# yoshitomo-matsubara/hnd-ghnd-object-detectors

Hardware: AMD Instinct MI355X
Metric: distill-step images/sec at 3x800x1333, GHND Faster R-CNN b3ch (higher is better)
Workload: dtype f32

## Files before the change

### hnd_ghnd_object_detectors_amd/csrc/conv_bx3.hip

```cpp

#include "bf16x3.h"
#include "common.h"

#include <stdlib.h>

namespace {

using hnd::bf8;
using hnd::cu_count;
using hnd::f32x4;
using hnd::FastDiv;
using hnd::split_pair;
using hnd::static_for;
using hnd::u32x4;

struct Bx3Args {
  FastDiv div_ow, div_oh;
  int nsl;
  int nchunks;
  int mrows;
  int cpg;
  int res_up;
};

template <int OFF>
__device__ __forceinline__ void rload(f32x4& dst, const float* p) {
  asm volatile("global_load_dwordx4 %0, %1, off offset:%2" : "=a"(dst) : "v"(p), "n"(OFF));
}
template <int CNT>
__device__ __forceinline__ void rwait(f32x4& a0, f32x4& a1, f32x4& a2, f32x4& a3, f32x4& a4, f32x4& a5, f32x4& a6,
                                      f32x4& a7) {
  asm volatile("s_waitcnt vmcnt(%8)"
               : "+a"(a0), "+a"(a1), "+a"(a2), "+a"(a3), "+a"(a4), "+a"(a5), "+a"(a6), "+a"(a7)
               : "n"(CNT));
}

__device__ __forceinline__ void bload(uint32_t& dst, const uint8_t* p) {
  asm volatile("global_load_ubyte %0, %1, off" : "=a"(dst) : "v"(p));
}
template <int CNT>
__device__ __forceinline__ void bwait8(uint32_t& a0, uint32_t& a1, uint32_t& a2, uint32_t& a3, uint32_t& a4, uint32_t& a5,
                                       uint32_t& a6, uint32_t& a7) {
  asm volatile("s_waitcnt vmcnt(%8)"
               : "+a"(a0), "+a"(a1), "+a"(a2), "+a"(a3), "+a"(a4), "+a"(a5), "+a"(a6), "+a"(a7)
               : "n"(CNT));
}

template <int CNT>
__device__ __forceinline__ void rwait8(f32x4& a0, f32x4& a1, f32x4& a2, f32x4& a3, f32x4& a4, f32x4& a5, f32x4& a6,
                                       f32x4& a7) {
  rwait<CNT>(a0, a1, a2, a3, a4, a5, a6, a7);
}

template <int KS, bool RES, bool MO, bool MK = false>
__global__ void __launch_bounds__(256, 1) bx3_kernel(const hnd_conv_desc d, const Bx3Args a) {
  static_assert(!MK || RES, "the mask build rides on the residual build's bookkeeping");
  constexpr int RESLOADS = RES ? (MK ? 32 : 16) : 0;
  constexpr int RING = RES ? 2 : 4, K = 32 * KS, MI = 4, NI = 4, PLANE = 64 * K, STORES = MO ? 32 : 16;
  static_assert(KS % RING == 0, "ring slots are compile-time: the ring must divide the k steps of a tile");
  extern __shared__ __attribute__((aligned(16))) uint16_t Bs[];
  const int tid = threadIdx.x, lane = tid & 63, wave = tid >> 6;
  const int l16 = lane & 15, g4 = lane >> 4;
  const int b = blockIdx.x, xcd = b & 7, idx = b >> 3, per_xcd = gridDim.x >> 3;
  const int slice = idx % a.nsl, tpx = per_xcd / a.nsl;
  const int team = xcd * tpx + idx / a.nsl, nteams = 8 * tpx;
  const int n0 = slice * 64;
  const int c_lo = (int)((long long)a.nchunks * team / nteams);
  const int c_hi = (int)((long long)a.nchunks * (team + 1) / nteams);

  auto a_ptr = [&](int cc, int mi) -> const float* {
    const unsigned m = min((unsigned)(cc * 64 + mi * 16 + l16), (unsigned)(a.mrows - 1));
    const unsigned t = hnd::fdiv(m, a.div_ow), ow_ = m - t * (unsigned)d.ow;
    const unsigned n_ = hnd::fdiv(t, a.div_oh), oh_ = t - n_ * (unsigned)d.oh;
    const size_t pix = ((size_t)n_ * d.h + oh_ * (unsigned)d.sh) * (size_t)d.w_ + ow_ * (unsigned)d.sw;
    return d.x + pix * (size_t)d.cin + (size_t)(g4 * 8);
  };
  const int col0 = n0 + l16 * 4;
  float es[NI], eb[NI];
#pragma unroll
  for (int ni = 0; ni < NI; ++ni) {
    es[ni] = d.epi_scale ? d.epi_scale[col0 + ni] : 1.f;
    eb[ni] = d.epi_shift ? d.epi_shift[col0 + ni] : 0.f;
  }
  const size_t slice_elems = (size_t)3 * PLANE;

  int c = c_lo;
  while (c < c_hi) {
    const int grp = a.cpg > 0 ? c / a.cpg : 0;
    const int seg_hi = a.cpg > 0 ? min(c_hi, (grp + 1) * a.cpg) : c_hi;
    __syncthreads();
    {
      const u32x4* src = (const u32x4*)(d.w_bf16x3 + ((size_t)grp * a.nsl + slice) * slice_elems);
      u32x4* dst = (u32x4*)Bs;
      constexpr int NV = 3 * PLANE / 8, UB = 12;
      static_assert(NV % (256 * UB) == 0, "slice does not divide among the threads");
#pragma unroll 1
      for (int i0 = 0; i0 < NV; i0 += 256 * UB) {
        u32x4 t[UB];
#pragma unroll
        for (int u = 0; u < UB; ++u) t[u] = src[i0 + u * 256 + tid];
#pragma unroll
        for (int u = 0; u < UB; ++u) dst[i0 + u * 256 + tid] = t[u];
      }
    }
    __syncthreads();

    int cc = c + wave;
    if (cc < seg_hi) {
      const float* aptr[MI];
      f32x4 ring[RING][MI][2];
#pragma unroll
      for (int mi = 0; mi < MI; ++mi) aptr[mi] = a_ptr(cc, mi);
      static_for<RING>([&](auto U) __attribute__((always_inline)) {
        constexpr int u = decltype(U)::value;
        static_for<MI>([&](auto I) __attribute__((always_inline)) {
          constexpr int mi = decltype(I)::value;
          rload<(u % KS) * 128>(ring[u][mi][0], aptr[mi]);
          rload<(u % KS) * 128 + 16>(ring[u][mi][1], aptr[mi]);
        });
      });
      uint32_t pl[2][3][MI][4];
      float dummy = 0.f;
#pragma unroll
      for (int i = 0; i < STORES; ++i) asm volatile("global_load_dword %0, %1, off" : "+v"(dummy) : "v"(aptr[0]));
      rwait<8 * (RING - 1) + STORES>(ring[0][0][0], ring[0][0][1], ring[0][1][0], ring[0][1][1], ring[0][2][0], ring[0][2][1],
                                     ring[0][3][0], ring[0][3][1]);
#pragma unroll
      for (int mi = 0; mi < MI; ++mi)
#pragma unroll
        for (int j = 0; j < 4; ++j) {
          const f32x4 v = ring[0][mi][j >> 1];
          const float x0 = (j & 1) ? v.z : v.x, x1 = (j & 1) ? v.w : v.y;
          split_pair(x0, x1, pl[0][0][mi][j], pl[0][1][mi][j], pl[0][2][mi][j]);
        }
      f32x4 acc[MI][NI];
      bf8 bfirst[3];
      {
        const uint16_t* br = Bs + l16 * K + ((g4 ^ l16) * 8);
        bfirst[0] = *(const bf8*)(br); bfirst[1] = *(const bf8*)(br + PLANE); bfirst[2] = *(const bf8*)(br + 2 * PLANE);
      }
      f32x4 resv[MI][4];
      uint32_t resm[MI][4];
      for (; cc < seg_hi; cc += 4) {
        const int cn = cc + 4 < seg_hi ? cc + 4 : cc;
        const float* nptr[MI];
#pragma unroll
        for (int mi = 0; mi < MI; ++mi) nptr[mi] = a_ptr(cn, mi);
        static_for<KS>([&](auto G) __attribute__((always_inline)) {
          constexpr int ks = decltype(G)::value, slot = ks % RING, par = ks & 1;
          constexpr int slot1 = (ks + 1) % RING;
          if constexpr (MK && ks == KS - 4) {
#pragma unroll
            for (int mi = 0; mi < MI; ++mi)
#pragma unroll
              for (int r = 0; r < 4; ++r)
                bload(resm[mi][r], d.mask_bits + (((size_t)min(cc * 64 + mi * 16 + g4 * 4 + r, a.mrows - 1) * (size_t)d.ldc + col0) >> 2));
          }
          if constexpr (RES && ks == KS - 4) {
#pragma unroll
            for (int mi = 0; mi < MI; ++mi) {
              const unsigned mr = (unsigned)(cc * 64 + mi * 16 + g4 * 4);
              const unsigned m0 = min(mr, (unsigned)(a.mrows - 4));
              const unsigned t = hnd::fdiv(m0, a.div_ow), ow_ = m0 - t * (unsigned)d.ow;
              const unsigned n_ = hnd::fdiv(t, a.div_oh), oh_ = t - n_ * (unsigned)d.oh;
              const size_t pu = ((size_t)n_ * d.res1_h + (oh_ >> 1)) * (size_t)d.res1_w + (ow_ >> 1);
              const bool up = a.res_up != 0;
              const unsigned ml = (unsigned)(a.mrows - 1);
              const size_t p0 = up ? pu : (size_t)min(mr, ml), p1 = up ? pu : (size_t)min(mr + 1, ml),
                           p2 = up ? pu + 1 : (size_t)min(mr + 2, ml), p3 = up ? pu + 1 : (size_t)min(mr + 3, ml);
              rload<0>(resv[mi][0], d.res1 + p0 * (size_t)d.ldc + col0);
              rload<0>(resv[mi][1], d.res1 + p1 * (size_t)d.ldc + col0);
              rload<0>(resv[mi][2], d.res1 + p2 * (size_t)d.ldc + col0);
              rload<0>(resv[mi][3], d.res1 + p3 * (size_t)d.ldc + col0);
            }
          }
          static_for<MI>([&](auto I) __attribute__((always_inline)) {
            constexpr int mi = decltype(I)::value;
            if constexpr (ks + RING < KS) {
              rload<(ks + RING) * 128>(ring[slot][mi][0], aptr[mi]);
              rload<(ks + RING) * 128 + 16>(ring[slot][mi][1], aptr[mi]);
            } else {
              rload<(ks + RING - KS) * 128>(ring[slot][mi][0], nptr[mi]);
              rload<(ks + RING - KS) * 128 + 16>(ring[slot][mi][1], nptr[mi]);
            }
          });
          constexpr int kResYounger = (RES && ks >= KS - 4 && ks <= KS - 4 + RING - 2) ? RESLOADS : 0;
          if constexpr (ks < RING - 1) {
            rwait<(8 * (RING - 1) + STORES + kResYounger < 63 ? 8 * (RING - 1) + STORES + kResYounger : 63)>(
                ring[slot1][0][0], ring[slot1][0][1], ring[slot1][1][0], ring[slot1][1][1], ring[slot1][2][0],
                ring[slot1][2][1], ring[slot1][3][0], ring[slot1][3][1]);
          } else {
            rwait<8 * (RING - 1) + kResYounger>(ring[slot1][0][0], ring[slot1][0][1], ring[slot1][1][0], ring[slot1][1][1],
                                                ring[slot1][2][0], ring[slot1][2][1], ring[slot1][3][0], ring[slot1][3][1]);
          }
          const int pos = ((ks * 4 + g4) ^ l16) * 8;
          bf8 bcur[3], bnxt[3];
          bcur[0] = bfirst[0]; bcur[1] = bfirst[1]; bcur[2] = bfirst[2];
          static_for<NI>([&](auto NIc) __attribute__((always_inline)) {
            constexpr int ni = decltype(NIc)::value;
            if constexpr (ni + 1 < NI) {
              const uint16_t* br = Bs + ((ni + 1) * 16 + l16) * K + pos;
              bnxt[0] = *(const bf8*)(br); bnxt[1] = *(const bf8*)(br + PLANE); bnxt[2] = *(const bf8*)(br + 2 * PLANE);
            } else {
              const uint16_t* br = Bs + l16 * K + ((((ks + 1) % KS) * 4 + g4) ^ l16) * 8;
              bfirst[0] = *(const bf8*)(br); bfirst[1] = *(const bf8*)(br + PLANE); bfirst[2] = *(const bf8*)(br + 2 * PLANE);
            }
            static_for<MI>([&](auto MIc) __attribute__((always_inline)) {
              constexpr int mi = decltype(MIc)::value;
              auto frag = [&](int q) __attribute__((always_inline)) {
                const u32x4 t = {pl[par][q][mi][0], pl[par][q][mi][1], pl[par][q][mi][2], pl[par][q][mi][3]};
                return __builtin_bit_cast(bf8, t);
              };
              const bf8 ah = frag(0), am = frag(1), al = frag(2);
              constexpr int p = ni * 4 + mi, rg = p >> 2, j = p & 3;
              const f32x4 v = ring[slot1][rg][j >> 1];
              const float x0 = (j & 1) ? v.z : v.x, x1 = (j & 1) ? v.w : v.y;
              f32x4 cacc = (ks == 0) ? f32x4{0.f, 0.f, 0.f, 0.f} : acc[mi][ni];
              cacc = __builtin_amdgcn_mfma_f32_16x16x32_bf16(al, bcur[0], cacc, 0, 0, 0);
              const uint32_t h0 = __float_as_uint(x0) & 0xffff0000u, h1 = __float_as_uint(x1) & 0xffff0000u;
              __builtin_amdgcn_sched_barrier(0);
              cacc = __builtin_amdgcn_mfma_f32_16x16x32_bf16(ah, bcur[2], cacc, 0, 0, 0);
              const float r0 = x0 - __uint_as_float(h0), r1 = x1 - __uint_as_float(h1);
              __builtin_amdgcn_sched_barrier(0);
              cacc = __builtin_amdgcn_mfma_f32_16x16x32_bf16(am, bcur[1], cacc, 0, 0, 0);
              const uint32_t m0 = __float_as_uint(r0) & 0xffff0000u, m1 = __float_as_uint(r1) & 0xffff0000u;
              __builtin_amdgcn_sched_barrier(0);
              cacc = __builtin_amdgcn_mfma_f32_16x16x32_bf16(am, bcur[0], cacc, 0, 0, 0);
              const float q0 = r0 - __uint_as_float(m0), q1 = r1 - __uint_as_float(m1);
              __builtin_amdgcn_sched_barrier(0);
              cacc = __builtin_amdgcn_mfma_f32_16x16x32_bf16(ah, bcur[1], cacc, 0, 0, 0);
              pl[par ^ 1][0][rg][j] = __builtin_amdgcn_perm(h1, h0, 0x07060302u);
              pl[par ^ 1][1][rg][j] = __builtin_amdgcn_perm(m1, m0, 0x07060302u);
              pl[par ^ 1][2][rg][j] = __builtin_amdgcn_perm(__float_as_uint(q1), __float_as_uint(q0), 0x07060302u);
              __builtin_amdgcn_sched_barrier(0);
              cacc = __builtin_amdgcn_mfma_f32_16x16x32_bf16(ah, bcur[0], cacc, 0, 0, 0);
              acc[mi][ni] = cacc;
              __builtin_amdgcn_sched_barrier(0);
            });
            if constexpr (ni + 1 < NI) { bcur[0] = bnxt[0]; bcur[1] = bnxt[1]; bcur[2] = bnxt[2]; }
          });
        });
        if constexpr (RES) {
          rwait8<32>(resv[0][0], resv[0][1], resv[0][2], resv[0][3], resv[1][0], resv[1][1], resv[1][2], resv[1][3]);
          rwait8<32>(resv[2][0], resv[2][1], resv[2][2], resv[2][3], resv[3][0], resv[3][1], resv[3][2], resv[3][3]);
          if constexpr (MK) {
            bwait8<32>(resm[0][0], resm[0][1], resm[0][2], resm[0][3], resm[1][0], resm[1][1], resm[1][2], resm[1][3]);
            bwait8<32>(resm[2][0], resm[2][1], resm[2][2], resm[2][3], resm[3][0], resm[3][1], resm[3][2], resm[3][3]);
          }
        }
#pragma unroll
        for (int mi = 0; mi < MI; ++mi)
#pragma unroll
          for (int r = 0; r < 4; ++r) {
            const size_t m = (size_t)min(cc * 64 + mi * 16 + g4 * 4 + r, a.mrows - 1);
            f32x4 v;
#pragma unroll
            for (int ni = 0; ni < NI; ++ni) {
              float x = acc[mi][ni][r] * es[ni] + eb[ni];
              if (RES) x += resv[mi][r][ni];
              if (MK) x = ((resm[mi][r] >> ni) & 1u) ? x : 0.f;
              v[ni] = d.relu ? fmaxf(x, 0.f) : x;
            }
            const size_t yo = m * (size_t)d.ldc + col0;
            *(f32x4*)(d.y + yo) = v;
            if (MO)
              d.mask_out[yo >> 2] = (uint8_t)((v[0] > 0.f ? 1 : 0) | (v[1] > 0.f ? 2 : 0) | (v[2] > 0.f ? 4 : 0) |
                                              (v[3] > 0.f ? 8 : 0));
          }
#pragma unroll
        for (int mi = 0; mi < MI; ++mi) aptr[mi] = nptr[mi];
      }
      asm volatile("s_waitcnt vmcnt(0)" : "+v"(dummy)::"memory");
    }
    c = seg_hi;
  }
}

__global__ void pack_bx3_kernel(const float* __restrict__ w, uint16_t* __restrict__ img, int rows_pad, int K, int KI, int groups,
                                long long group_stride, long long total) {
  const int nsl = rows_pad / 64;
  const size_t plane = (size_t)64 * KI;
  for (long long e = blockIdx.x * (long long)blockDim.x + threadIdx.x; e < total; e += (long long)gridDim.x * blockDim.x) {
    const int k = (int)(e % K);
    long long t = e / K;
    const int row = (int)(t % rows_pad), g = (int)(t / rows_pad);
    const float x = w[(size_t)g * (size_t)group_stride + (size_t)row * K + k];
    const uint32_t xb = __float_as_uint(x), hb = xb & 0xffff0000u;
    const float r1 = x - __uint_as_float(hb);
    const uint32_t mb = __float_as_uint(r1) & 0xffff0000u;
    const float r2 = r1 - __uint_as_float(mb);
    const int part = k / KI, kk = k - part * KI;
    const int s = row / 64, r = row % 64, c = kk >> 3, pos = c ^ (r & 15);
    uint16_t* o = img + (((size_t)part * groups + g) * nsl + s) * 3 * plane + (size_t)r * KI + pos * 8 + (kk & 7);
    o[0] = (uint16_t)(hb >> 16);
    o[plane] = (uint16_t)(mb >> 16);
    o[2 * plane] = (uint16_t)(__float_as_uint(r2) >> 16);
  }
}

template <int KS, bool RES, bool MO, bool MK = false>
int launch_bx3_t(const hnd_conv_desc& d, const Bx3Args& a, int grid, hipStream_t stream) {
  const size_t lds = (size_t)3 * 64 * 32 * KS * sizeof(uint16_t);
  return hnd::launch_big_lds<bx3_kernel<KS, RES, MO, MK>>(dim3(grid), dim3(256), lds, 160 * 1024, stream, "hnd_conv2d_igemm(bx3)",
                                                          d, a);
}

}

namespace hnd {

static bool bx3_recommended(long long rows_per_image, int kdim, int cout) {
  if (rows_per_image <= 0 || cout <= 0 || cout % 64 != 0) return false;
  if (kdim != 128 && (kdim % 256 != 0 || kdim > 2048)) return false;
  const long long nteams = team_count(cout, 64);
  if (nteams == 0) return false;
  const long long chunks_at_16 = (rows_per_image * 16 + 63) / 64;
  return chunks_at_16 / nteams >= (kdim > 512 ? 16 : 8);
}

bool bx3_applies(const hnd_conv_desc& d) {
  if (!d.w_bf16x3) return false;
  if (d.kh != 1 || d.kw != 1 || d.bh != 0 || d.bw != 0 || d.cin != d.kdim) return false;
  if (d.kdim != 128 && (d.kdim % 256 != 0 || d.kdim > 2048)) return false;
  if (d.stats || d.pro_scale || d.res2 || d.mask || d.bwd_x) return false;
  if (d.mask_bits && d.mask_out) return false;
  if (d.mask_bits && d.kdim <= 256 && (!d.res1 || d.res1_mode != 0)) return false;
  if (d.res1 && ((uintptr_t)d.res1 % 16) != 0) return false;
  if (d.res1 && d.res1_mode == 1 && (d.yh != 2 * d.res1_h || d.yw != 2 * d.res1_w || d.ow % 4 != 0)) return false;
  if (d.cout % 64 != 0 || d.ldc % 4 != 0 || ((uintptr_t)d.y % 16) != 0) return false;
  if (team_count(d.cout, 64) == 0) return false;
  if (d.y_sh != 1 || d.y_sw != 1 || d.y_oh != 0 || d.y_ow != 0 || d.yh != d.oh || d.yw != d.ow) return false;
  if (!samples_inside(d)) return false;
  const long long M = gemm_rows(d);
  if (M < 64 || d.w_group_rows % 64 != 0) return false;
  if (M % 64 != 0 && d.w_group_rows != 0) return false;
  return true;
}

static int launch_bx3_one(const hnd_conv_desc& d, int kpart, hipStream_t stream) {
  Bx3Args a;
  a.div_ow = make_fastdiv((unsigned)d.ow);
  a.div_oh = make_fastdiv((unsigned)d.oh);
  a.nsl = d.cout / 64;
  a.mrows = (int)gemm_rows(d);
  a.nchunks = (a.mrows + 63) / 64;
  a.cpg = d.w_group_rows / 64;
  a.res_up = d.res1 && d.res1_mode == 1;
  const int grid = (cu_count() / 8) * 8;
  if (d.mask_bits)
    return kpart == 128 ? launch_bx3_t<4, true, false, true>(d, a, grid, stream)
                        : launch_bx3_t<8, true, false, true>(d, a, grid, stream);
  const int sel = (kpart == 128 ? 0 : 4) | (d.res1 ? 2 : 0) | (d.mask_out ? 1 : 0);
  switch (sel) {
    case 0: return launch_bx3_t<4, false, false>(d, a, grid, stream);
    case 1: return launch_bx3_t<4, false, true>(d, a, grid, stream);
    case 2: return launch_bx3_t<4, true, false>(d, a, grid, stream);
    case 3: return launch_bx3_t<4, true, true>(d, a, grid, stream);
    case 4: return launch_bx3_t<8, false, false>(d, a, grid, stream);
    case 5: return launch_bx3_t<8, false, true>(d, a, grid, stream);
    case 6: return launch_bx3_t<8, true, false>(d, a, grid, stream);
    default: return launch_bx3_t<8, true, true>(d, a, grid, stream);
  }
}

int launch_bx3_tiled(const hnd_conv_desc& d, int mi, hipStream_t stream);

static const int BX3_TILED_BELOW_K128 = 3, BX3_TILED_BELOW_K256 = 3, BX3_TILED_BELOW_K512 = 10, BX3_TILED_BELOW_KLONG = 16;
static const int BX3_TILED_128_ROWS_FROM = 10;

int bx3_build(const hnd_conv_desc& d) {
  const long long chunks = (gemm_rows(d) + 63) / 64, nteams = team_count(d.cout, 64);
  const long long per_team = (chunks + nteams - 1) / nteams;
  const bool is_long = d.kdim >= 1024;
  const int rows = is_long && per_team >= BX3_TILED_128_ROWS_FROM ? 2 : 1;
  const int forced = debug_picker("bx3_tiled");
  if (forced >= 0) {
    const int mi = debug_picker("bx3_tiled_mi");
    return forced ? (mi == 1 || mi == 2 ? mi : rows) : 0;
  }
  if (d.w_group_rows > 0) return 0;
  const int below = d.kdim <= 128 ? BX3_TILED_BELOW_K128
                                  : (d.kdim <= 256 ? BX3_TILED_BELOW_K256 : (is_long ? BX3_TILED_BELOW_KLONG : BX3_TILED_BELOW_K512));
  return per_team < below ? rows : 0;
}

int launch_bx3(const hnd_conv_desc& d, int build, hipStream_t stream) {
  if (build) return launch_bx3_tiled(d, build, stream);
  if (d.kdim <= 256) return launch_bx3_one(d, d.kdim, stream);
  const long long groups = d.w_group_rows > 0 ? gemm_rows(d) / d.w_group_rows : 1;
  const int parts = d.kdim / 256;
  const size_t part_elems = (size_t)groups * (size_t)(d.cout / 64) * (size_t)3 * 64 * 256;
  for (int p = 0; p < parts; ++p) {
    hnd_conv_desc q = d;
    if (p + 1 < parts) {
      q.relu = 0;
      q.mask_out = nullptr;
      q.mask_bits = nullptr;
    }
    if (p > 0) {
      q.x = d.x + (size_t)256 * p;
      q.w_bf16x3 = d.w_bf16x3 + part_elems * (size_t)p;
      q.epi_shift = nullptr;
      q.res1 = d.y;
      q.res1_mode = 0;
    }
    const int rc = launch_bx3_one(q, 256, stream);
    if (rc) return rc;
  }
  return 0;
}

}

extern "C" int hnd_bf16x3_recommended(int64_t rows_per_image, int kdim, int cout) {
  return hnd::bx3_recommended((long long)rows_per_image, kdim, cout) ? 1 : 0;
}

extern "C" size_t hnd_pack_bf16x3_elems(int rows_pad, int kdim, int groups) {
  if (rows_pad <= 0 || rows_pad % 64 != 0 || kdim <= 0 || kdim % 8 != 0 || groups < 1) return 0;
  return (size_t)groups * (size_t)rows_pad * (size_t)kdim * 3;
}

extern "C" int hnd_pack_bf16x3(const float* w_packed, uint16_t* img, int rows_pad, int kdim, int groups,
                               int64_t group_stride, void* stream) {
  HND_REQUIRE(w_packed && img && rows_pad > 0 && rows_pad % 64 == 0 && (kdim == 128 || (kdim % 256 == 0 && kdim <= 2048)) &&
                  groups >= 1 && (groups == 1 || group_stride >= (int64_t)rows_pad * kdim),
              "hnd_pack_bf16x3: bad arguments (kdim must be 128 or a multiple of 256 up to 2048)");
  const long long total = (long long)groups * rows_pad * kdim;
  long long blocks = (total + 255) / 256;
  if (blocks > 8192) blocks = 8192;
  hipLaunchKernelGGL(pack_bx3_kernel, dim3((unsigned)blocks), dim3(256), 0, hnd::as_stream(stream), w_packed, img, rows_pad,
                     kdim, kdim > 256 ? 256 : kdim, groups, (long long)group_stride, total);
  return hnd::check_launch("hnd_pack_bf16x3");
}
```

### hnd_ghnd_object_detectors_amd/csrc/conv_bx3_tiled.hip

```cpp
#include "bf16x3.h"
#include "common.h"

namespace {

using hnd::bf8;
using hnd::f32x4;
using hnd::FastDiv;
using hnd::u32x4;

struct Bx3tArgs {
  FastDiv div_ow, div_oh;
  int nsl;
  int mrows;
  int cpg;
  int tpg;
  int ngroups;
  int res_up;
};

template <int MI>
__global__ void __launch_bounds__(256, MI == 1 ? 3 : 2) bx3t_kernel(const hnd_conv_desc d, const Bx3tArgs a) {
  constexpr int NI = 4, KP = 64, PPLANE = 64 * KP, PBUF = 3 * PPLANE, NB = PBUF / 8 / 256;
  __shared__ __attribute__((aligned(16))) uint16_t Bs[2][PBUF];
  const int tid = threadIdx.x, lane = tid & 63, wave = tid >> 6;
  const int l16 = lane & 15, g4 = lane >> 4;
  const int lb = hnd::xcd_contiguous_block();
  const int rt = lb / a.nsl, slice = lb - rt * a.nsl;
  int grp = 0, row0 = rt * 64 * MI, mlim = a.mrows;
  if (a.tpg > 0) {
    grp = rt / a.tpg;
    row0 = (grp * a.cpg + (rt - grp * a.tpg) * MI) * 64;
    mlim = min((grp + 1) * a.cpg * 64, a.mrows);
  }
  const int wrow0 = row0 + wave * 16 * MI;
  const int KI = d.kdim == 128 ? 128 : 256, ppp = KI / KP, npieces = d.kdim / KP;
  const size_t slice_elems = (size_t)3 * 64 * KI;
  const int col0 = slice * 64 + l16 * 4;

  const float* ap[MI];
#pragma unroll
  for (int mi = 0; mi < MI; ++mi) {
    const unsigned m = (unsigned)min(wrow0 + mi * 16 + l16, mlim - 1);
    const unsigned t = hnd::fdiv(m, a.div_ow), ow_ = m - t * (unsigned)d.ow;
    const unsigned n_ = hnd::fdiv(t, a.div_oh), oh_ = t - n_ * (unsigned)d.oh;
    const size_t pix = ((size_t)n_ * d.h + oh_ * (unsigned)d.sh) * (size_t)d.w_ + ow_ * (unsigned)d.sw;
    ap[mi] = d.x + pix * (size_t)d.cin + (size_t)(g4 * 8);
  }
  float es[NI], eb[NI];
#pragma unroll
  for (int ni = 0; ni < NI; ++ni) {
    es[ni] = d.epi_scale ? d.epi_scale[col0 + ni] : 1.f;
    eb[ni] = d.epi_shift ? d.epi_shift[col0 + ni] : 0.f;
  }

  u32x4 bt[NB];
  f32x4 acur[MI][2][2];
  auto load_b = [&](int pc) __attribute__((always_inline)) {
    const int part = pc / ppp, pin = pc - part * ppp;
    const uint16_t* base = d.w_bf16x3 + (((size_t)part * a.ngroups + grp) * a.nsl + slice) * slice_elems;
#pragma unroll
    for (int u = 0; u < NB; ++u) {
      const int idx = u * 256 + tid, plane = idx >> 9, row = (idx >> 3) & 63, cl = idx & 7;
      bt[u] = *(const u32x4*)(base + (size_t)plane * 64 * KI + row * KI + (((pin * 8 + cl) ^ (row & 15)) * 8));
    }
  };
  auto store_b = [&](int buf) __attribute__((always_inline)) {
#pragma unroll
    for (int u = 0; u < NB; ++u) {
      const int idx = u * 256 + tid, plane = idx >> 9, row = (idx >> 3) & 63, cl = idx & 7;
      *(u32x4*)(&Bs[buf][plane * PPLANE + row * KP + ((cl ^ ((row >> 1) & 7)) * 8)]) = bt[u];
    }
  };
  auto load_a = [&](int pc, int ksl) __attribute__((always_inline)) {
#pragma unroll
    for (int mi = 0; mi < MI; ++mi) {
      acur[mi][ksl][0] = *(const f32x4*)(ap[mi] + pc * KP + ksl * 32);
      acur[mi][ksl][1] = *(const f32x4*)(ap[mi] + pc * KP + ksl * 32 + 4);
    }
  };

  load_b(0);
  load_a(0, 0);
  load_a(0, 1);
  store_b(0);
  __syncthreads();

  f32x4 acc[MI][NI], run[MI][NI];
#pragma unroll
  for (int mi = 0; mi < MI; ++mi)
#pragma unroll
    for (int ni = 0; ni < NI; ++ni) run[mi][ni] = f32x4{0.f, 0.f, 0.f, 0.f};

  int pin = 0, part = 0;
#pragma unroll 1
  for (int pc = 0; pc < npieces; ++pc) {
    const bool more = pc + 1 < npieces;
    if (more) load_b(pc + 1);
    if (pin == 0) {
#pragma unroll
      for (int mi = 0; mi < MI; ++mi)
#pragma unroll
        for (int ni = 0; ni < NI; ++ni) acc[mi][ni] = f32x4{0.f, 0.f, 0.f, 0.f};
    }
    const uint16_t* B = Bs[pc & 1];
#pragma unroll
    for (int ksl = 0; ksl < 2; ++ksl) {
      bf8 ah[MI], am[MI], al[MI];
#pragma unroll
      for (int mi = 0; mi < MI; ++mi) {
        u32x4 h, m, l;
#pragma unroll
        for (int j = 0; j < 4; ++j) {
          const f32x4 v = acur[mi][ksl][j >> 1];
          const float x0 = (j & 1) ? v.z : v.x, x1 = (j & 1) ? v.w : v.y;
          uint32_t hp, mp, lp;
          hnd::split_pair(x0, x1, hp, mp, lp);
          h[j] = hp; m[j] = mp; l[j] = lp;
        }
        ah[mi] = __builtin_bit_cast(bf8, h);
        am[mi] = __builtin_bit_cast(bf8, m);
        al[mi] = __builtin_bit_cast(bf8, l);
      }
      if (more) load_a(pc + 1, ksl);
#pragma unroll
      for (int ni = 0; ni < NI; ++ni) {
        const int row = ni * 16 + l16;
        const uint16_t* br = B + row * KP + (((ksl * 4 + g4) ^ ((row >> 1) & 7)) * 8);
        const bf8 bh = *(const bf8*)(br), bm = *(const bf8*)(br + PPLANE), bl = *(const bf8*)(br + 2 * PPLANE);
#pragma unroll
        for (int mi = 0; mi < MI; ++mi) {
          f32x4 c = acc[mi][ni];
          c = __builtin_amdgcn_mfma_f32_16x16x32_bf16(al[mi], bh, c, 0, 0, 0);
          c = __builtin_amdgcn_mfma_f32_16x16x32_bf16(ah[mi], bl, c, 0, 0, 0);
          c = __builtin_amdgcn_mfma_f32_16x16x32_bf16(am[mi], bm, c, 0, 0, 0);
          c = __builtin_amdgcn_mfma_f32_16x16x32_bf16(am[mi], bh, c, 0, 0, 0);
          c = __builtin_amdgcn_mfma_f32_16x16x32_bf16(ah[mi], bm, c, 0, 0, 0);
          c = __builtin_amdgcn_mfma_f32_16x16x32_bf16(ah[mi], bh, c, 0, 0, 0);
          acc[mi][ni] = c;
        }
      }
    }
    if (more) store_b((pc + 1) & 1);
    if (++pin == ppp) {
      pin = 0;
      const bool first = part == 0;
      ++part;
#pragma unroll
      for (int mi = 0; mi < MI; ++mi)
#pragma unroll
        for (int r = 0; r < 4; ++r) {
          f32x4 rv = {0.f, 0.f, 0.f, 0.f};
          bool add = !first;
          if (first) {
            add = d.res1 != nullptr;
            if (add) {
              const unsigned m = (unsigned)min(wrow0 + mi * 16 + g4 * 4 + r, mlim - 1);
              size_t p = m;
              if (a.res_up) {
                const unsigned t = hnd::fdiv(m, a.div_ow), ow_ = m - t * (unsigned)d.ow;
                const unsigned n_ = hnd::fdiv(t, a.div_oh), oh_ = t - n_ * (unsigned)d.oh;
                p = ((size_t)n_ * d.res1_h + (oh_ >> 1)) * (size_t)d.res1_w + (ow_ >> 1);
              }
              rv = *(const f32x4*)(d.res1 + p * (size_t)d.ldc + col0);
            }
          } else {
#pragma unroll
            for (int ni = 0; ni < NI; ++ni) rv[ni] = run[mi][ni][r];
          }
#pragma unroll
          for (int ni = 0; ni < NI; ++ni) {
            float x = acc[mi][ni][r] * es[ni] + (first ? eb[ni] : 0.f);
            if (add) x += rv[ni];
            run[mi][ni][r] = x;
          }
        }
    }
    __syncthreads();
  }

#pragma unroll
  for (int mi = 0; mi < MI; ++mi)
#pragma unroll
    for (int r = 0; r < 4; ++r) {
      const int m = wrow0 + mi * 16 + g4 * 4 + r;
      if (m >= mlim) continue;
      const size_t yo = (size_t)m * (size_t)d.ldc + col0;
      uint32_t mk = 0xfu;
      if (d.mask_bits) mk = d.mask_bits[yo >> 2];
      f32x4 v;
#pragma unroll
      for (int ni = 0; ni < NI; ++ni) {
        float x = run[mi][ni][r];
        x = ((mk >> ni) & 1u) ? x : 0.f;
        v[ni] = d.relu ? fmaxf(x, 0.f) : x;
      }
      *(f32x4*)(d.y + yo) = v;
      if (d.mask_out)
        d.mask_out[yo >> 2] =
            (uint8_t)((v[0] > 0.f ? 1 : 0) | (v[1] > 0.f ? 2 : 0) | (v[2] > 0.f ? 4 : 0) | (v[3] > 0.f ? 8 : 0));
    }
}

template <int MI>
int launch_bx3t_t(const hnd_conv_desc& d, hipStream_t stream) {
  Bx3tArgs a;
  a.div_ow = hnd::make_fastdiv((unsigned)d.ow);
  a.div_oh = hnd::make_fastdiv((unsigned)d.oh);
  a.nsl = d.cout / 64;
  a.mrows = (int)((long long)d.n * d.oh * d.ow);
  a.cpg = d.w_group_rows / 64;
  a.res_up = d.res1 && d.res1_mode == 1;
  const int nchunks = (a.mrows + 63) / 64;
  long long row_tiles;
  if (a.cpg > 0) {
    a.ngroups = nchunks / a.cpg;
    a.tpg = (a.cpg + MI - 1) / MI;
    row_tiles = (long long)a.ngroups * a.tpg;
  } else {
    a.ngroups = 1;
    a.tpg = 0;
    row_tiles = (nchunks + MI - 1) / MI;
  }
  const long long grid = row_tiles * a.nsl;
  if (grid <= 0 || grid >= (1ll << 31)) {
    hnd::set_error("launch_bx3_tiled: grid of %lld tiles", grid);
    return HND_ERR_INVALID;
  }
  hipLaunchKernelGGL(bx3t_kernel<MI>, dim3((unsigned)grid), dim3(256), 0, stream, d, a);
  return hnd::check_launch("hnd_conv2d_igemm(bx3 tiled)");
}

}

namespace hnd {

int launch_bx3_tiled(const hnd_conv_desc& d, int mi, hipStream_t stream) {
  return mi == 1 ? launch_bx3t_t<1>(d, stream) : launch_bx3t_t<2>(d, stream);
}

}
```

### hnd_ghnd_object_detectors_amd/ops.py

```python
import ctypes as C
import os
import math

import torch

from . import _lib
from ._lib import ConvDesc, WgradDesc, MsePair, MimicPair, MIMIC_KINDS, check

_L = _lib.load()
PARAM_EPOCH = [0]


def stream_ptr():
    return torch.cuda.current_stream().cuda_stream


def ptr(t):
    return None if t is None else t.data_ptr()


def round_up(x, m):
    return (x + m - 1) // m * m


def chan_pad_of(c):
    return 4 if c <= 4 else round_up(c, 32)


def sync_check():
    check(_L.hnd_sync_check(stream_ptr()), 'hnd_sync_check')


def device_arch():
    return (_L.hnd_device_arch() or b'').decode()


BX3_MODE = ['policy' if os.environ.get('HND_BF16X3', '1') != '0' else 'off']


def bx3_on():
    return BX3_MODE[0] != 'off'


class emulation(object):

    def __init__(self, mode):
        assert mode in ('policy', 'off', 'force', 'bx3', 'bxs'), mode
        self.mode = mode

    def __enter__(self):
        self.saved, BX3_MODE[0] = BX3_MODE[0], self.mode
        return self

    def __exit__(self, *exc):
        BX3_MODE[0] = self.saved
        return False


def emulation_unless(allowed):
    import contextlib
    return contextlib.nullcontext() if allowed else emulation('off')


def bxs_recommended(rows_per_image, kdim, cout, taps):
    return bool(_L.hnd_bf16x3s_recommended(int(rows_per_image), int(kdim), int(cout), int(taps)))


def bx3_recommended(rows_per_image, kdim, cout):
    return bool(_L.hnd_bf16x3_recommended(int(rows_per_image), int(kdim), int(cout)))


def bx3_image(buf, rows_pad, kdim, groups=1, group_stride=0, out=None, force=None):
    if out is None:
        out = torch.empty(int(_L.hnd_pack_bf16x3_elems(rows_pad, kdim, groups)), dtype=torch.int16, device=buf.device)
    check(_L.hnd_pack_bf16x3(buf.data_ptr(), out.data_ptr(), rows_pad, kdim, groups, int(group_stride), stream_ptr()),
          'hnd_pack_bf16x3')
    return out


def bxs_image(buf, rows_pad, kdim, groups=1, group_stride=0, out=None, force=None):
    if out is None:
        out = torch.empty(int(_L.hnd_pack_bf16x3s_elems(rows_pad, kdim, groups)), dtype=torch.int16, device=buf.device)
    check(_L.hnd_pack_bf16x3s(buf.data_ptr(), out.data_ptr(), rows_pad, kdim, groups, int(group_stride), stream_ptr()),
          'hnd_pack_bf16x3s')
    return out


class PackedWeight(object):
    groups, group_stride, taps, bx3, bxs = 1, 0, 1, None, None

    def __init__(self, buf, rows, kdim, chan_pad, chan_real=None, groups=1, group_stride=0, taps=1):
        self.buf, self.rows, self.rows_pad, self.kdim = buf, rows, round_up(rows, 64), kdim
        self.chan_pad, self.chan_real = chan_pad, chan_pad if chan_real is None else chan_real
        self.groups, self.group_stride, self.taps = groups, group_stride, taps
        self.bx3 = self.bxs = None

    def fill(self):
        """(re)compute buf from the source weight (nothing to do for a buffer the caller filled)"""

    def repack(self):
        self.fill()
        self.refresh_images()

    def refresh_images(self):
        if self.bx3 is not None:
            bx3_image(self.buf, self.rows_pad, self.kdim, self.groups, self.group_stride, out=self.bx3)
        if self.bxs is not None:
            bxs_image(self.buf, self.rows_pad, self.kdim, self.groups, self.group_stride, out=self.bxs)

    def can_bx3(self):
        return (self.taps == 1 and self.kdim == self.chan_pad and self.rows_pad % 64 == 0
                and (self.kdim == 128 or (self.kdim % 256 == 0 and self.kdim <= 2048)))

    def can_bxs(self):
        return (self.groups == 1 and self.kdim % 128 == 0 and self.chan_pad % 64 == 0 and self.rows_pad % 64 == 0
                and self.kdim == self.taps * self.chan_pad)

    def attach(self, which):
        if which == 'bx3':
            if self.bx3 is None and self.can_bx3():
                self.bx3 = bx3_image(self.buf, self.rows_pad, self.kdim, self.groups, self.group_stride)
            return self.bx3
        if self.bxs is None and self.can_bxs():
            self.bxs = bxs_image(self.buf, self.rows_pad, self.kdim, self.groups, self.group_stride)
        return self.bxs


class DirectWeights(PackedWeight):
    def __init__(self, w, transposed=False, chan_pad=None, taps=None, kscale=None):
        cout, cin, kh, kw = w.shape
        assert w.is_contiguous() and w.dtype == torch.float32
        if taps is None:
            taps = (0, 1, kh, 0, 1, kw)
        i0, istep, ni, j0, jstep, nj = taps
        chans = cout if transposed else cin
        rows = cin if transposed else cout
        if chan_pad is None:
            chan_pad = chan_pad_of(chans)
        kdim = round_up(ni * nj * chan_pad, 32)
        PackedWeight.__init__(self, torch.empty(round_up(rows, 64) * kdim, dtype=torch.float32, device=w.device), rows,
                              kdim, chan_pad, chans, taps=ni * nj)
        self.src, self.kscale = w, kscale
        self.args = (cout, cin, kh, kw, int(transposed), chan_pad, i0, istep, ni, j0, jstep, nj)
        self.repack()

    def repack(self):
        if PACK_BATCH['open'] and self.kscale is None:
            PACK_BATCH['items'].append(self)
        else:
            PackedWeight.repack(self)

    def fill(self):
        check(_L.hnd_pack_weights(self.src.data_ptr(), self.buf.data_ptr(), *self.args, stream_ptr()), 'hnd_pack_weights')
        if self.kscale is not None:
            check(_L.hnd_scale_packed_k(self.buf.data_ptr(), self.rows_pad, self.kdim, self.taps, self.chan_pad,
                                        self.kscale.data_ptr(), min(self.kscale.numel(), self.chan_pad), stream_ptr()),
                  'hnd_scale_packed_k')


pack_weights = DirectWeights


PACK_BATCH = {'open': False, 'items': []}


def pack_batch_begin():
    PACK_BATCH['open'], PACK_BATCH['items'] = True, []


def pack_batch_end():
    from ._lib import PackDesc
    items, PACK_BATCH['open'], PACK_BATCH['items'] = PACK_BATCH['items'], False, []
    if not items:
        return
    arr = (PackDesc * len(items))()
    for d, pw in zip(arr, items):
        d.src, d.dst = pw.src.data_ptr(), pw.buf.data_ptr()
        (d.cout, d.cin, d.kh, d.kw, d.transposed, d.chan_pad, d.i0, d.istep, d.ni, d.j0, d.jstep, d.nj) = pw.args
    check(_L.hnd_pack_weights_batched(arr, len(items), stream_ptr()), 'hnd_pack_weights_batched')
    for pw in items:
        pw.refresh_images()


def fbn_fold(weight, bias, mean, var, eps=0.0, cs=None, out=None):
    c = weight.numel()
    cs = cs or c
    if out is not None:
        scale, shift = out
        assert scale.numel() == cs and shift.numel() == cs
    else:
        scale = torch.empty(cs, dtype=torch.float32, device=weight.device)
        shift = torch.empty(cs, dtype=torch.float32, device=weight.device)
    check(_L.hnd_fbn_fold(ptr(weight), ptr(bias), ptr(mean), ptr(var), ptr(scale), ptr(shift), c, cs, float(eps),
                          stream_ptr()), 'hnd_fbn_fold')
    return scale, shift


class ConvLaunch(object):
    __slots__ = ('desc', 'ref', 'keep', 'flops', 'alg_flops', 'variant', 'build', 'relay')

    def __init__(self, desc, keep, flops=0):
        self.desc, self.keep, self.flops = desc, keep, flops
        self.alg_flops = flops
        self.ref = C.byref(desc)
        self.relay = None
        self.refresh_variant()

    def refresh_variant(self):
        need = int(_L.hnd_conv2d_igemm_workspace(self.ref))
        if need == 0:
            self.relay, self.desc.relay_ws = None, None
        elif self.relay is None or self.relay.numel() * 4 < need:
            self.relay = torch.zeros((need + 3) // 4, dtype=torch.float32, device=torch.device('cuda', torch.cuda.current_device()))
            self.desc.relay_ws = self.relay.data_ptr()
        tile = _L.hnd_conv2d_igemm_tile(self.ref)
        self.variant = ('stem7_lds' if tile == 9 else 'igemm_c4_128x64') if self.desc.cin == 4 else \
            ('igemm_128x128', 'igemm_128x64', 'igemm_64x128', 'igemm_64x64', 'thin_n4', 'bres_128',
             'bres_64', 'bres2_128', 'bres2_64', 'stem7_lds', 'unused', 'bstream_128', 'bstream_64', 'bx3_64',
             'bxs_128', 'bxs_64')[tile]
        self.build = ('persistent', 'tiled')[int(_L.hnd_conv2d_igemm_build(self.ref))] if tile == 13 else None

    def run(self, stream=None):
        rc = _L.hnd_conv2d_igemm(self.ref, stream if stream is not None else stream_ptr())
        if rc:
            check(rc, 'hnd_conv2d_igemm')


def _nhwc(t):
    assert t.dim() == 4 and t.is_contiguous() and t.dtype == torch.float32, (t.shape, t.stride(), t.dtype)
    return t.shape


def conv_desc(x, pw, y, *, kh, kw, oh, ow, sh, dh, bh, sw, dw, bw, cout, y_sh=1, y_oh=0, y_sw=1, y_ow=0,
              pro_scale=None, pro_shift=None, pro_relu=False, epi_scale=None, epi_shift=None, res1=None,
              res1_up=False, res2=None, mask=None, relu=False, stats=None, mask_bits=None, mask_out=None,
              bwd_stats=None, rows_per_image=None, w_group_rows=0):
    n, h, w, cin = _nhwc(x)
    ny, yh, yw, ldc = _nhwc(y)
    assert ny == n and pw.kdim >= kh * kw * cin and pw.chan_pad == cin, (pw.kdim, kh, kw, cin, pw.chan_pad)
    assert (pw.groups > 1) == (w_group_rows > 0), (pw.groups, w_group_rows)
    if pro_scale is not None and pro_shift is None:
        pro_shift = _zeros(cin, x.device)
    d = ConvDesc()
    d.x, d.w, d.y = ptr(x), ptr(pw.buf), ptr(y)
    d.pro_scale, d.pro_shift = ptr(pro_scale), ptr(pro_shift)
    d.epi_scale, d.epi_shift = ptr(epi_scale), ptr(epi_shift)
    d.res1, d.res2, d.mask, d.stats = ptr(res1), ptr(res2), ptr(mask), ptr(stats)
    d.n, d.h, d.w_, d.cin = n, h, w, cin
    d.oh, d.ow, d.yh, d.yw, d.cout, d.ldc = oh, ow, yh, yw, cout, ldc
    d.y_sh, d.y_oh, d.y_sw, d.y_ow = y_sh, y_oh, y_sw, y_ow
    d.kh, d.kw = kh, kw
    d.sh, d.dh, d.bh, d.sw, d.dw, d.bw = sh, dh, bh, sw, dw, bw
    d.kdim = pw.kdim
    d.w_group_rows, d.w_group_stride = w_group_rows, pw.group_stride
    d.pro_relu, d.relu = int(pro_relu), int(relu)
    if res1 is not None and res1_up:
        d.res1_mode, d.res1_h, d.res1_w = 1, res1.shape[1], res1.shape[2]
        assert res1.shape[0] == n and res1.shape[3] == ldc
    elif res1 is not None:
        assert tuple(res1.shape) == tuple(y.shape)
    for t in (res2, mask):
        assert t is None or tuple(t.shape) == tuple(y.shape)
    for t in (mask_bits, mask_out):
        assert t is None or (t.dtype == torch.uint8 and t.is_contiguous() and ldc % 4 == 0
                             and tuple(t.shape) == (ny, yh, yw, ldc // 4)), (None if t is None else t.shape, y.shape)
    assert mask is None or mask_bits is None
    d.mask_bits, d.mask_out = ptr(mask_bits), ptr(mask_out)
    rpi, mode = oh * ow if rows_per_image is None else rows_per_image, BX3_MODE[0]
    if mode in ('force', 'bx3') or (mode == 'policy' and bx3_recommended(rpi, pw.kdim, cout)):
        d.w_bf16x3 = ptr(pw.attach('bx3'))
    if mode in ('force', 'bxs') or (mode == 'policy' and bxs_recommended(rpi, pw.kdim, cout, kh * kw)):
        d.w_bf16x3s = ptr(pw.attach('bxs'))
    if stats is not None:
        assert stats.numel() >= stats_tiles(n * oh * ow) * 2 * cout
    if bwd_stats is not None:
        bx, bsc, bsh, bmu, brs, brelu = bwd_stats
        assert stats is not None and tuple(bx.shape) == tuple(y.shape) and cout == ldc
        assert res1 is None and res2 is None and mask is None and mask_bits is None and not relu
        assert min(t.numel() for t in (bsc, bsh, bmu, brs)) >= ldc
        d.bwd_x, d.bwd_scale, d.bwd_shift, d.bwd_mean, d.bwd_rstd = ptr(bx), ptr(bsc), ptr(bsh), ptr(bmu), ptr(brs)
        d.bwd_relu = int(brelu)
    keep = (x, pw, y, pro_scale, pro_shift, epi_scale, epi_shift, res1, res2, mask, stats, mask_bits, mask_out,
            bwd_stats)
    return ConvLaunch(d, keep, flops=2 * n * oh * ow * min(cout, pw.rows) * kh * kw * min(cin, pw.chan_real))


_ZEROS = {}


def _zeros(n, device):
    key = (n, str(device))
    if key not in _ZEROS:
        _ZEROS[key] = torch.zeros(n, dtype=torch.float32, device=device)
    return _ZEROS[key]


def stats_tiles(m):
    return (m + 127) // 128


def conv_out_size(h, k, stride, pad):
    return (h + 2 * pad - k) // stride + 1


def conv_forward(x, pw, y, k, stride=1, pad=0, **kw_):
    kh, kwid = (k, k) if isinstance(k, int) else k
    n, h, w, cin = x.shape
    oh, ow = conv_out_size(h, kh, stride, pad), conv_out_size(w, kwid, stride, pad)
    assert (y.shape[1], y.shape[2]) == (oh, ow), (y.shape, oh, ow)
    cout = kw_.pop('cout', y.shape[3])
    assert cout <= round_up(pw.rows, 64)
    return conv_desc(x, pw, y, kh=kh, kw=kwid, oh=oh, ow=ow, sh=stride, dh=1, bh=-pad, sw=stride, dw=1, bw=-pad,
                     cout=cout, **kw_)


def dgrad_tap_classes(k, stride, pad):
    out = []
    for ph in range(stride):
        i0 = (ph + pad) % stride
        ni = len(range(i0, k, stride))
        bh = (ph + pad - i0) // stride
        out.append((i0, stride, ni, bh))
    return out


def conv_dgrad(dy, w_param, dx, k, stride=1, pad=0, accumulate=False, fold_scale=None, **kw_):
    n, h, w, ldc = dx.shape
    cache = None
    if not isinstance(w_param, torch.Tensor):
        cache, w_param = w_param, w_param.weight
    cout_w, cin_w, kh, kwid = w_param.shape
    assert kh == k and kwid == k and dy.shape[3] == chan_pad_of(cout_w)
    launches, packs = [], []
    classes = dgrad_tap_classes(k, stride, pad)
    for ph, (i0, istep, ni, bh) in enumerate(classes):
        for pw_, (j0, jstep, nj, bw) in enumerate(classes):
            if ni == 0 or nj == 0:
                assert accumulate, 'tap-less output parity: caller must accumulate into a defined dx'
                continue
            ohv, owv = len(range(ph, h, stride)), len(range(pw_, w, stride))
            if ohv == 0 or owv == 0:
                continue
            taps = (i0, istep, ni, j0, jstep, nj)
            if cache is not None:
                pk = cache.get(True, dy.shape[3], taps, kscale=fold_scale)
            else:
                pk = pack_weights(w_param, transposed=True, chan_pad=dy.shape[3], taps=taps, kscale=fold_scale)
            packs.append(pk)
            extra = dict(kw_)
            if accumulate:
                extra['res1'] = dx
            launches.append(conv_desc(dy, pk, dx, kh=ni, kw=nj, oh=ohv, ow=owv, sh=1, dh=-1, bh=bh, sw=1, dw=-1,
                                      bw=bw, cout=ldc, y_sh=stride, y_oh=ph, y_sw=stride,
                                      y_ow=pw_, **extra))
    return launches, packs


class WgradLaunch(object):
    __slots__ = ('desc', 'ref', 'keep', 'flops', 'alg_flops', 'variant')

    def __init__(self, desc, keep, flops):
        self.desc, self.keep, self.flops = desc, keep, flops
        self.alg_flops = flops
        self.ref = C.byref(desc)
        self.variant = {1: 'stem7_wgrad', 2: 'thin_wgrad', 3: 'wgrad_ring'}.get(
            int(_L.hnd_conv2d_wgrad_variant(self.ref)), 'wgrad_m128' if desc.cout >= 128 else 'wgrad_m64')

    def run(self, stream=None):
        rc = _L.hnd_conv2d_wgrad(self.ref, stream if stream is not None else stream_ptr())
        if rc:
            check(rc, 'hnd_conv2d_wgrad')


def conv_wgrad(x, dy, dw, k, stride=1, pad=0, pro_scale=None, pro_shift=None, pro_relu=False, splitk=0,
               slabs=None):
    n, h, w, cin = _nhwc(x)
    _, oh, ow, ldy = _nhwc(dy)
    cout, cin_real, kh, kwid = dw.shape
    assert dw.is_contiguous() and kh == k and kwid == k
    d = WgradDesc()
    d.x, d.dy, d.dw = ptr(x), ptr(dy), ptr(dw)
    d.pro_scale, d.pro_shift, d.pro_relu = ptr(pro_scale), ptr(pro_shift), int(pro_relu)
    d.n, d.h, d.w_, d.cin, d.cin_real = n, h, w, cin, cin_real
    d.oh, d.ow, d.cout, d.ldy = oh, ow, cout, ldy
    d.kh, d.kw, d.stride, d.pad, d.splitk = k, k, stride, pad, splitk
    need = _L.hnd_conv2d_wgrad_workspace(C.byref(d))
    if slabs is None or slabs.numel() * 4 < need:
        slabs = torch.empty((need + 3) // 4, dtype=torch.float32, device=x.device)
    d.slabs = ptr(slabs)
    return WgradLaunch(d, (x, dy, dw, slabs, pro_scale, pro_shift), 2 * n * oh * ow * cout * k * k * cin_real)


def wgrad_workspace_of(desc):
    return int(_L.hnd_conv2d_wgrad_workspace(C.byref(desc)))


def wgrad_workspace_bytes(n, h, w, cin, oh, ow, cout, k, stride, pad):
    d = WgradDesc()
    d.n, d.h, d.w_, d.cin, d.cin_real, d.oh, d.ow, d.cout, d.ldy = n, h, w, cin, cin, oh, ow, cout, chan_pad_of(cout)
    d.kh, d.kw, d.stride, d.pad = k, k, stride, pad
    return _L.hnd_conv2d_wgrad_workspace(C.byref(d))


def transform_image(src, dst, index, out_h, out_w, rscale_h, rscale_w, mean, std):
    c, h, w = src.shape
    assert c == 3 and src.is_contiguous() and dst.shape[3] == 4
    m = (C.c_float * 3)(*mean)
    s = (C.c_float * 3)(*std)
    _hbm('transform_image', 12 * h * w + 16 * dst.shape[1] * dst.shape[2], lambda: check(
        _L.hnd_transform_image(ptr(src), h, w, ptr(dst), index, out_h, out_w, dst.shape[1], dst.shape[2],
                               float(rscale_h), float(rscale_w), m, s, stream_ptr()), 'hnd_transform_image'))


def transform_image_u8(src, dst, index, out_h, out_w, rscale_h, rscale_w, mean, std, hwc, flip=False):
    assert src.dtype == torch.uint8 and src.is_contiguous() and src.dim() == 3 and dst.shape[3] == 4
# ... 600 lines not shown
```

Before: 215.0.

## Extend bf16x3 1x1 conv path to K=64, masked K=128, and res2 residual

Allows the split-bf16x3 matrix-core 1x1 convolution path to handle K=64 weights with an 8-wide XOR swizzle. It also routes masked K=128 convolutions through the tiled kernel and accepts a res2 residual by remapping it onto res1. The aim is to move more of the ResNet bottleneck 1x1 convolutions off the slower fallback convolution kernels. Coverage is controlled by a class bitmask whose default enables only the res2-residual case, so K=64 and masked K=128 stay off unless a debug override is set. The widened eligibility checks add the risk of wrong results or mis-selection on edge shapes.

```diff
diff --git a/hnd_ghnd_object_detectors_amd/csrc/conv_bx3.hip b/hnd_ghnd_object_detectors_amd/csrc/conv_bx3.hip
--- a/hnd_ghnd_object_detectors_amd/csrc/conv_bx3.hip
+++ b/hnd_ghnd_object_detectors_amd/csrc/conv_bx3.hip
@@ -290,7 +290,7 @@
     const uint32_t mb = __float_as_uint(r1) & 0xffff0000u;
     const float r2 = r1 - __uint_as_float(mb);
     const int part = k / KI, kk = k - part * KI;
-    const int s = row / 64, r = row % 64, c = kk >> 3, pos = c ^ (r & 15);
+    const int s = row / 64, r = row % 64, c = kk >> 3, pos = c ^ (r & (KI == 64 ? 7 : 15));
     uint16_t* o = img + (((size_t)part * groups + g) * nsl + s) * 3 * plane + (size_t)r * KI + pos * 8 + (kk & 7);
     o[0] = (uint16_t)(hb >> 16);
     o[plane] = (uint16_t)(mb >> 16);
@@ -309,8 +309,21 @@
 
 namespace hnd {
 
+static const int BX3_SMALLK_DEFAULT = 8;
+static int bx3_smallk_classes() {
+  const int v = debug_picker("bx3_smallk");
+  return v >= 0 ? v : BX3_SMALLK_DEFAULT;
+}
+static int bx3_k64_class(int cout) { return cout == 256 ? 1 : (cout == 64 ? 2 : 0); }
+static const long long BX3_K64_MIN_ROWS_PER_IMAGE = 16384;
+static bool bx3_k64_recommended(long long rows_per_image, int cout) {
+  if (team_count(cout, 64) == 0 || rows_per_image < BX3_K64_MIN_ROWS_PER_IMAGE) return false;
+  return (bx3_smallk_classes() & bx3_k64_class(cout)) != 0;
+}
+
 static bool bx3_recommended(long long rows_per_image, int kdim, int cout) {
   if (rows_per_image <= 0 || cout <= 0 || cout % 64 != 0) return false;
+  if (kdim == 64) return bx3_k64_recommended(rows_per_image, cout);
   if (kdim != 128 && (kdim % 256 != 0 || kdim > 2048)) return false;
   const long long nteams = team_count(cout, 64);
   if (nteams == 0) return false;
@@ -318,13 +331,28 @@
   return chunks_at_16 / nteams >= (kdim > 512 ? 16 : 8);
 }
 
+static bool bx3_res2_is_residual(const hnd_conv_desc& d) {
+  return d.res2 && !d.res1 && d.mask_bits && d.cout == 2 * d.kdim && (bx3_smallk_classes() & 8);
+}
+
+static bool bx3_tiled_only(const hnd_conv_desc& d) {
+  if (d.kdim == 64) return true;
+  const bool dense_res = bx3_res2_is_residual(d) || (d.res1 && d.res1_mode == 0);
+  return d.kdim == 128 && d.mask_bits && !dense_res;
+}
+
 bool bx3_applies(const hnd_conv_desc& d) {
   if (!d.w_bf16x3) return false;
   if (d.kh != 1 || d.kw != 1 || d.bh != 0 || d.bw != 0 || d.cin != d.kdim) return false;
-  if (d.kdim != 128 && (d.kdim % 256 != 0 || d.kdim > 2048)) return false;
-  if (d.stats || d.pro_scale || d.res2 || d.mask || d.bwd_x) return false;
+  if (d.kdim != 64 && d.kdim != 128 && (d.kdim % 256 != 0 || d.kdim > 2048)) return false;
+  if (d.stats || d.pro_scale || d.mask || d.bwd_x) return false;
+  if (d.res2 && (!bx3_res2_is_residual(d) || ((uintptr_t)d.res2 % 16) != 0)) return false;
   if (d.mask_bits && d.mask_out) return false;
-  if (d.mask_bits && d.kdim <= 256 && (!d.res1 || d.res1_mode != 0)) return false;
+  const bool tiled_only = bx3_tiled_only(d);
+  if (tiled_only) {
+    if (!(bx3_smallk_classes() & (d.kdim == 64 ? bx3_k64_class(d.cout) : 4)) || debug_picker("bx3_tiled") == 0) return false;
+  }
+  if (d.mask_bits && d.kdim <= 256 && !tiled_only && !d.res2 && (!d.res1 || d.res1_mode != 0)) return false;
   if (d.res1 && ((uintptr_t)d.res1 % 16) != 0) return false;
   if (d.res1 && d.res1_mode == 1 && (d.yh != 2 * d.res1_h || d.yw != 2 * d.res1_w || d.ow % 4 != 0)) return false;
   if (d.cout % 64 != 0 || d.ldc % 4 != 0 || ((uintptr_t)d.y % 16) != 0) return false;
@@ -332,7 +360,7 @@
   if (d.y_sh != 1 || d.y_sw != 1 || d.y_oh != 0 || d.y_ow != 0 || d.yh != d.oh || d.yw != d.ow) return false;
   if (!samples_inside(d)) return false;
   const long long M = gemm_rows(d);
-  if (M < 64 || d.w_group_rows % 64 != 0) return false;
+  if (M < (tiled_only ? 1 : 64) || d.w_group_rows % 64 != 0) return false;
   if (M % 64 != 0 && d.w_group_rows != 0) return false;
   return true;
 }
@@ -374,17 +402,24 @@
   const bool is_long = d.kdim >= 1024;
   const int rows = is_long && per_team >= BX3_TILED_128_ROWS_FROM ? 2 : 1;
   const int forced = debug_picker("bx3_tiled");
-  if (forced >= 0) {
+  if (forced > 0 || bx3_tiled_only(d)) {
     const int mi = debug_picker("bx3_tiled_mi");
-    return forced ? (mi == 1 || mi == 2 ? mi : rows) : 0;
-  }
+    return mi == 1 || mi == 2 ? mi : rows;
+  }
+  if (forced == 0) return 0;
   if (d.w_group_rows > 0) return 0;
   const int below = d.kdim <= 128 ? BX3_TILED_BELOW_K128
                                   : (d.kdim <= 256 ? BX3_TILED_BELOW_K256 : (is_long ? BX3_TILED_BELOW_KLONG : BX3_TILED_BELOW_K512));
   return per_team < below ? rows : 0;
 }
 
-int launch_bx3(const hnd_conv_desc& d, int build, hipStream_t stream) {
+int launch_bx3(const hnd_conv_desc& d0, int build, hipStream_t stream) {
+  hnd_conv_desc d = d0;
+  if (d.res2) {
+    d.res1 = d.res2;
+    d.res1_mode = 0;
+    d.res2 = nullptr;
+  }
   if (build) return launch_bx3_tiled(d, build, stream);
   if (d.kdim <= 256) return launch_bx3_one(d, d.kdim, stream);
   const long long groups = d.w_group_rows > 0 ? gemm_rows(d) / d.w_group_rows : 1;
@@ -423,9 +458,10 @@
 
 extern "C" int hnd_pack_bf16x3(const float* w_packed, uint16_t* img, int rows_pad, int kdim, int groups,
                                int64_t group_stride, void* stream) {
-  HND_REQUIRE(w_packed && img && rows_pad > 0 && rows_pad % 64 == 0 && (kdim == 128 || (kdim % 256 == 0 && kdim <= 2048)) &&
-                  groups >= 1 && (groups == 1 || group_stride >= (int64_t)rows_pad * kdim),
-              "hnd_pack_bf16x3: bad arguments (kdim must be 128 or a multiple of 256 up to 2048)");
+  HND_REQUIRE(w_packed && img && rows_pad > 0 && rows_pad % 64 == 0 &&
+                  (kdim == 64 || kdim == 128 || (kdim % 256 == 0 && kdim <= 2048)) && groups >= 1 &&
+                  (groups == 1 || group_stride >= (int64_t)rows_pad * kdim),
+              "hnd_pack_bf16x3: bad arguments (kdim must be 64, 128 or a multiple of 256 up to 2048)");
   const long long total = (long long)groups * rows_pad * kdim;
   long long blocks = (total + 255) / 256;
   if (blocks > 8192) blocks = 8192;
diff --git a/hnd_ghnd_object_detectors_amd/csrc/conv_bx3_tiled.hip b/hnd_ghnd_object_detectors_amd/csrc/conv_bx3_tiled.hip
--- a/hnd_ghnd_object_detectors_amd/csrc/conv_bx3_tiled.hip
+++ b/hnd_ghnd_object_detectors_amd/csrc/conv_bx3_tiled.hip
@@ -33,7 +33,7 @@
     mlim = min((grp + 1) * a.cpg * 64, a.mrows);
   }
   const int wrow0 = row0 + wave * 16 * MI;
-  const int KI = d.kdim == 128 ? 128 : 256, ppp = KI / KP, npieces = d.kdim / KP;
+  const int KI = d.kdim <= 128 ? d.kdim : 256, ppp = KI / KP, npieces = d.kdim / KP, xm = KI == 64 ? 7 : 15;
   const size_t slice_elems = (size_t)3 * 64 * KI;
   const int col0 = slice * 64 + l16 * 4;
 
@@ -61,7 +61,7 @@
 #pragma unroll
     for (int u = 0; u < NB; ++u) {
       const int idx = u * 256 + tid, plane = idx >> 9, row = (idx >> 3) & 63, cl = idx & 7;
-      bt[u] = *(const u32x4*)(base + (size_t)plane * 64 * KI + row * KI + (((pin * 8 + cl) ^ (row & 15)) * 8));
+      bt[u] = *(const u32x4*)(base + (size_t)plane * 64 * KI + row * KI + (((pin * 8 + cl) ^ (row & xm)) * 8));
     }
   };
   auto store_b = [&](int buf) __attribute__((always_inline)) {
diff --git a/hnd_ghnd_object_detectors_amd/ops.py b/hnd_ghnd_object_detectors_amd/ops.py
--- a/hnd_ghnd_object_detectors_amd/ops.py
+++ b/hnd_ghnd_object_detectors_amd/ops.py
@@ -110,7 +110,7 @@
 
     def can_bx3(self):
         return (self.taps == 1 and self.kdim == self.chan_pad and self.rows_pad % 64 == 0
-                and (self.kdim == 128 or (self.kdim % 256 == 0 and self.kdim <= 2048)))
+                and (self.kdim in (64, 128) or (self.kdim % 256 == 0 and self.kdim <= 2048)))
 
     def can_bxs(self):
         return (self.groups == 1 and self.kdim % 128 == 0 and self.chan_pad % 64 == 0 and self.rows_pad % 64 == 0
```

After: 215.6, median of 2. No clear change (+0.3%).
